# GuyTevet/motion-diffusion-model

Measured on AMD Instinct MI355X. Metric: motions/sec (B=128, T=196, 50-step DDPM), higher is better.
Workload: dtype f16x3 (fp32 operands split into fp16 hi+lo, 3 fp16 MFMA products, fp32 accumulate; everything else fp32); 1 GPU; HumanML3D text2motion, 50-step p_sample_loop with CFG 2.5 (2 denoiser forwards per step), batch=128 per GPU, T=196, 8-layer d=512 trans_enc MDM, random-init weights, cached text embedding; global_batch=128, diffusion_steps=50, parallelism=dp1: batch shards, no data-path collective, all_gather of final samples

## Files before the change

include/mdm_hip.h:

```cpp
#ifndef MDM_HIP_H
#define MDM_HIP_H

#include <stddef.h>
#include <stdint.h>

#ifdef __cplusplus
extern "C" {
#endif

#define MDM_OK 0
#define MDM_EINVAL (-1)
#define MDM_ESTATE (-2)
#define MDM_ENOSPC (-3)
#define MDM_EHIP (-4)
#define MDM_EUNSUPPORTED (-5)

#define MDM_ABI_VERSION 10

typedef struct mdm_model mdm_model_t;

#define MDM_ARCH_TRANS_ENC 0
#define MDM_ARCH_TRANS_DEC 1

typedef struct mdm_config {
// ... 3 lines not shown
  int32_t ff_size;
  int32_t num_layers;
  int32_t num_heads;
  int32_t clip_dim;
  int32_t max_len;
  int32_t mask_frames;
  int32_t arch;
  int32_t context_len;
} mdm_config_t;

int mdm_abi_version(void);
const char* mdm_build_info(void);
const char* mdm_last_error(void);

int mdm_create(const mdm_config_t* cfg, mdm_model_t** out);
void mdm_destroy(mdm_model_t* m);

#define MDM_OPT_SMALL_GEMM_MAX_SEQS 1
#define MDM_OPT_SMALL_GEMM_ROW_TILES 2
#define MDM_OPT_DEC_FUSED_XATTN 3
#define MDM_OPT_DEC_FUSED_SELFATTN 4
#define MDM_OPT_ATTN_DIRECT_OUT 5
#define MDM_OPT_DEC_TIME_TOKEN 6
int mdm_set_option(mdm_model_t* m, int32_t key, int32_t value);
int mdm_get_option(const mdm_model_t* m, int32_t key, int32_t* value);

int mdm_set_time_add(mdm_model_t* m, const float* add_dev, int32_t B);

int mdm_set_weight(mdm_model_t* m, const char* name, const float* dev_ptr, int64_t numel);

size_t mdm_const_bytes(const mdm_model_t* m);
int mdm_prepare(mdm_model_t* m, void* const_ws_dev, size_t const_ws_bytes, void* stream);

int mdm_weights_in_range(mdm_model_t* m, int32_t* in_range, void* stream);

#define MDM_PREC_F32 0
#define MDM_PREC_F16X3 1
int mdm_set_precision(mdm_model_t* m, int32_t mode);

size_t mdm_workspace_bytes(const mdm_model_t* m, int32_t nseq, int32_t nframes);

#define MDM_BRANCH_COND 0
#define MDM_BRANCH_UNCOND 1
#define MDM_BRANCH_BOTH 2

int mdm_forward(mdm_model_t* m, const float* x_dev, const int64_t* timesteps_dev, const float* text_embed_dev,
// ... 133 lines not shown
```

motion-diffusion-model_amd/_native.py:

```python
import ctypes as C
import os

_HERE = os.path.dirname(os.path.abspath(__file__))
LIB_NAME = "libmdm_hip.so"
LIB_PATH = os.path.join(_HERE, "csrc", LIB_NAME)
PROBE_LIB_PATH = os.path.join(_HERE, "csrc", "libmdm_hip_probe.so")

MDM_OK = 0
BRANCH_COND, BRANCH_UNCOND, BRANCH_BOTH = 0, 1, 2
ACT_NONE, ACT_GELU, ACT_SILU = 0, 1, 2
PRECISIONS = {"f32": 0, "f16x3": 1}
PROF_CLASSES = ("linear", "attention", "layernorm", "embed", "outproj", "elementwise")

EXPORTED_SYMBOLS = [
    "mdm_abi_version", "mdm_build_info", "mdm_last_error", "mdm_create", "mdm_destroy", "mdm_set_weight", "mdm_const_bytes",
    "mdm_prepare", "mdm_workspace_bytes", "mdm_forward", "mdm_sampler_step", "mdm_randn", "mdm_sample_loop",
    "mdm_linear", "mdm_layernorm", "mdm_attention", "mdm_profile_enable", "mdm_profile_read", "mdm_profile_reset",
    "mdm_set_precision", "mdm_linear_x3", "mdm_linear_x3_scratch_bytes", "mdm_attention_x3", "mdm_attention_x3_scratch_bytes",
    "mdm_recover_from_ric", "mdm_workspace_bytes_dec", "mdm_forward_dec", "mdm_workspace_bytes_dec_loop",
    "mdm_sample_loop_dec", "mdm_weights_in_range", "mdm_set_option", "mdm_get_option", "mdm_set_time_add",
    "mdm_rot6d_to_smpl_joints", "mdm_smpl_workspace_bytes", "mdm_smpl_forward",
]
PROBE_SYMBOLS = ["mdm_debug_set", "mdm_debug_get", "mdm_linear_f16f6", "mdm_linear_f16f6_scratch_bytes", "mdm_probe_in_proj"]
ABI_VERSION = 10
OPTIONS = {"small_gemm_max_seqs": 1, "small_gemm_row_tiles": 2, "dec_fused_xattn": 3, "dec_fused_selfattn": 4, "attn_direct_out": 5,
           "dec_time_token": 6}
ARCH = {"trans_enc": 0, "trans_dec": 1}


class MdmConfig(C.Structure):
    _fields_ = [(n, C.c_int32) for n in ("njoints", "nfeats", "latent_dim", "ff_size", "num_layers", "num_heads",
                                         "clip_dim", "max_len", "mask_frames", "arch", "context_len")]


class MdmSmplModel(C.Structure):
    _fields_ = [(n, C.c_void_p) for n in ("j0", "jdirs", "blend", "weights_t", "sel_blend", "sel_weights_t", "extra_t")] + \
               [("parents", C.POINTER(C.c_int32))] + [(n, C.c_int32) for n in ("J", "V", "n_sel", "n_extra")]


class MdmSmplCall(C.Structure):
    _fields_ = [(n, C.c_int32) for n in ("pose_rep", "glob", "translation", "vertstrans", "n_points", "root_point")] + \
               [("point_map", C.POINTER(C.c_int32)), ("glob_rot_mat", C.POINTER(C.c_float)), ("beta1", C.c_float)]


SMPL_POSE_REPS = {"rot6d": 0, "rotvec": 1, "rotmat": 2, "rotquat": 3}
SMPL_REP_FEATS = {"rot6d": 6, "rotvec": 3, "rotmat": 9, "rotquat": 4}


class MdmStep(C.Structure):
# ... 127 lines not shown
```

motion-diffusion-model_amd/csrc/api_launch.h:

```cpp
#pragma once

namespace {

struct Workspace {
  float *tok, *qkv, *att, *ffn, *cond;
  QkvPlanes qp;
  p16_t *xah, *xal;
  float *stat1, *stat2;
  p16_t *tokh, *tokl;
  p16_t *atth, *attl;
  p16_t *ffnh, *ffnl;
  size_t bytes;
};

Workspace carve(const mdm_model* m, int nseq, int T, void* base) {
  const size_t D = m->cfg.latent_dim, FF = m->cfg.ff_size, S = (size_t)T + 1, M = (size_t)nseq * S;
  size_t off = 0;
  auto take = [&](size_t floats) {
    size_t o = off;
    off += align_up(floats * sizeof(float), 256);
    return base ? reinterpret_cast<float*>(static_cast<char*>(base) + o) : nullptr;
  };
  Workspace w;
  w.tok = take(M * D);
// ... 217 lines not shown
    RowMajorLoader bl{w, K, N, K};
    launch_gemm_f32(al, bl, ep, M, N, K, s, x3);
  }
  return rt_launch_status();
}

int launch_linear_x3(Profiler* pf, X3Operand a, X3Weights w, const float* bias, const float* res, float* out,
                     p16_t* oh, p16_t* ol, int M, int N, int K, int act, int scale_cols, float col_scale, int seq_len,
                     hipStream_t s, X3Operand res_planes = X3Operand{nullptr, nullptr}) {
  if (K % X3_BK != 0) return fail(MDM_EINVAL, "f16x3 linear: K must be a multiple of 32");
  if (N % 4 != 0) return fail(MDM_EINVAL, "f16x3 linear: N must be a multiple of 4");
  ProfScope ps(pf, MDM_PROF_LINEAR, 2.0 * M * (double)N * K, s);
  X3Epilogue ep{out, bias, res, res_planes.hi, res_planes.lo, oh, ol, N, scale_cols, col_scale, QkvPlanes{}, 0, 0,
                nullptr, nullptr, nullptr, nullptr, nullptr, nullptr, 1, 1.f, 1, 1, 1};
#ifdef MDM_PROBES
  if (g_x3_delay > 1) ep.emb_B = g_x3_delay;
#endif
  const int rc = launch_gemm_x3(a, w, ep, M, N, K, act, seq_len, s, g_x3_ablate);
  if (rc == -2) return fail(MDM_EUNSUPPORTED, "f16x3 linear: unsupported (activation, residual, output) combination");
  return rt_launch_status();
}

int launch_in_proj_x3(Profiler* pf, X3Operand a, X3Weights w, const float* bias, const QkvPlanes& qp, int nseq, int S,
                      int D, float qscale, hipStream_t s) {
  if (D % X3_BK != 0) return fail(MDM_EINVAL, "f16x3 in_proj: latent_dim must be a multiple of 32");
  ProfScope ps(pf, MDM_PROF_LINEAR, 2.0 * nseq * S * 3.0 * D * (double)D, s);
  X3Epilogue ep{nullptr, bias, nullptr, nullptr, nullptr, nullptr, nullptr, 3 * D, D, qscale, qp, S, D,
                nullptr, nullptr, nullptr, nullptr, nullptr, nullptr, 1, 1.f, 1, 1, 1};
  const int rc = launch_gemm_x3_qkv(a, w, ep, nseq, S, D, s);
  if (rc == -2) return fail(MDM_EUNSUPPORTED, "f16x3 in_proj: sequences longer than 224 tokens");
  return rt_launch_status();
}

struct LnArgs {
  const float* astat = nullptr; const float* colsum = nullptr;
  X3Operand res{nullptr, nullptr}; const float* rstat = nullptr; const float* rgamma = nullptr; const float* rbeta = nullptr;
  float* ostat = nullptr;
  int parts = 1; float inv_dim = 1.f;
  const float* res_f32 = nullptr; int emb_T = 1, emb_B = 1, emb_nbranch = 1;
  bool small = false;
  X3sShape shape{1, 1};
  int stat_cols = 256;
};
inline bool use_small_gemm(const mdm_model* m, int nseq, int S) {
  return m->precision == MDM_PREC_F16X3 && m->lnfold && (nseq <= m->x3s.max_seqs || S > X3_TM) &&
         m->cfg.latent_dim % 128 == 0 && m->cfg.latent_dim % 256 == 0 && m->cfg.ff_size % 256 == 0;
}
int launch_x3_ln(Profiler* pf, int prof_cat, int kind, X3Operand a, X3Weights w, const float* bias, const LnArgs& ln,
                 float* out, p16_t* oh, p16_t* ol, const QkvPlanes* qp, int M, int N, int K, int S, int D,
                 int scale_cols, float col_scale, hipStream_t s) {
  if (K % X3_BK != 0 || N % 4 != 0) return fail(MDM_EINVAL, "f16x3 linear: K % 32 and N % 4 must be 0");
  if (ln.parts < 1 || ln.parts > (ln.small ? 8 : 4)) return fail(MDM_EUNSUPPORTED, "folded LayerNorm: too many partial sums per row (D <= 1024)");
  ProfScope ps(pf, prof_cat, 2.0 * M * (double)N * K, s);
// ... 52 lines not shown
```

motion-diffusion-model_amd/csrc/api_runtime.h:

```cpp
#pragma once

namespace {

thread_local std::string g_err;
#ifdef MDM_PROBES
int g_x3_ablate = 0;
int g_x3_reuse_planes = 0;
int g_f6_reference = 0;
int g_x3_delay = 0;
#else
constexpr int g_x3_ablate = 0, g_x3_reuse_planes = 0;
#endif

int fail(int code, const std::string& msg) {
  g_err = msg;
  return code;
}

#ifdef MDM_EMU
inline int rt_launch_status() { return 0; }
inline int rt_copy(void* dst, const void* src, size_t bytes, hipStream_t) { memcpy(dst, src, bytes); return 0; }
template <class K> inline int rt_allow_lds(K, size_t) { return 0; }
#else
inline int rt_launch_status() {
// ... 96 lines not shown
  const float* time_add_next = nullptr;
  int time_add_B = 0;
  const float* time_add = nullptr;
  bool dec_time_token = false;
  int jf = 0, jf_pad = 0;
  int precision = MDM_PREC_F16X3;
  struct LayerPlanes { X3Weights in_proj, out_proj, linear1, linear2; };
  std::vector<LayerPlanes> planes;
  struct LayerFold { X3Weights in_proj, linear1; float *c_qkv, *b_qkv, *c_1, *b_1; };
  std::vector<LayerFold> fold;
  struct DecFold { float *w_in, *c_in, *b_in, *w_q, *c_q, *b_q, *w_1, *c_1, *b_1; };
  std::vector<DecFold> dec_fold;
  struct DecPlanes { X3Weights in_proj, out_proj, q, out_proj2, linear1, linear2; };
  std::vector<DecPlanes> dec_planes;
  X3Weights in_planes{nullptr, nullptr};
  int jf_k = 0;
  X3Weights out_planes_f{nullptr, nullptr};
  float *c_out = nullptr, *b_out = nullptr;
  float *wkv_all = nullptr, *bkv_all = nullptr;
  bool lnfold = false;
  X3sOptions x3s;
  int fused_xattn = 3;
  bool fused_selfattn = true;
  bool attn_direct = false;
  X3Weights out_planes{nullptr, nullptr};
  float* out_bias_pad = nullptr;
  int jf_out = 0;

  const float* W(const std::string& k) const { return w.at(k); }
  const float* L(int layer, const char* suffix) const {
    return w.at((cfg.arch == MDM_ARCH_TRANS_DEC ? "seqTransDecoder.layers." : "seqTransEncoder.layers.") +
                std::to_string(layer) + "." + suffix);
  }
};

namespace {

#ifdef MDM_EMU
struct ChainGuard { explicit ChainGuard(void*) {} };
#else
struct DeviceChain {
  std::mutex mu;
  hipEvent_t ev = nullptr;
  hipStream_t last = nullptr;
  bool has = false;
};
// ... 57 lines not shown
```

motion-diffusion-model_amd/csrc/encoder.h:

```cpp
#pragma once

namespace {

int embed_frames_x3(mdm_model* m, const Workspace& ws, const float* x, int B, int T, int nbranch, hipStream_t s, const CondTokArgs& ct) {
  const int D = m->cfg.latent_dim, KP = m->jf_k;
  ProfScope ps(&m->prof, MDM_PROF_EMBED, 2.0 * B * T * (double)D * m->jf, s);
  p16_t* ph = reinterpret_cast<p16_t*>(ws.ffn);
  p16_t* pl = ph + (size_t)B * T * KP;
  MDM_LAUNCH(pose_planes_cond_kernel, dim3(((T + 31) / 32) * (KP / 32) * B + nbranch * B), dim3(256), 0, s, x, ph, pl, T, m->jf, KP, B, ct);
  if (int rc = rt_launch_status()) return rc;
  LnArgs a;
  a.res_f32 = m->W("sequence_pos_encoder.pe");
  a.emb_T = T; a.emb_B = B; a.emb_nbranch = nbranch;
  a.small = use_small_gemm(m, nbranch * B, T + 1) && KP == 288;
  a.shape = x3s_shape(m->x3s, nbranch * B);
  return launch_x3_ln(nullptr, MDM_PROF_EMBED, 5, X3Operand{ph, pl}, m->in_planes, m->W("input_process.poseEmbedding.bias"), a,
                      nullptr, ws.tokh, ws.tokl, nullptr, B * T, D, KP, T + 1, D, 0, 1.f, s);
}
inline bool use_embed_x3(const mdm_model* m, int T) {
  return m->precision == MDM_PREC_F16X3 && x3_waves_setting() == 8 &&
         (T + 1 <= X3_TM || (use_small_gemm(m, 1, T + 1) && m->jf_k == 288));
}

int embed_tokens(mdm_model* m, const Workspace& ws, const float* x, const long long* timesteps,
// ... 22 lines not shown
  return rt_launch_status();
}

int encoder(mdm_model* m, const Workspace& ws, int nseq, int B, int S, const int* lengths, hipStream_t s) {
  Profiler* pf = &m->prof;
  const int D = m->cfg.latent_dim, FF = m->cfg.ff_size, H = m->cfg.num_heads, M = nseq * S;
  const float qscale = 1.0f / sqrtf((float)(D / H));
  if (m->precision == MDM_PREC_F16X3 && m->lnfold && x3_waves_setting() == 8 && (S <= X3_TM || use_small_gemm(m, nseq, S))) {
    const X3Operand xb{ws.tokh, ws.tokl}, xa{ws.xah, ws.xal}, attp{ws.atth, ws.attl}, ffnp{ws.ffnh, ws.ffnl};
    const bool small = use_small_gemm(m, nseq, S);
    const X3sShape shape = x3s_shape(m->x3s, nseq);
    const int scols = small ? x3s_tn(shape.ncb) : 256;
    const int parts = (D + scols - 1) / scols;
    const float inv_dim = 1.0f / (float)D;
    auto LN = [&]() { LnArgs a; a.small = small; a.shape = shape; a.stat_cols = scols; a.parts = parts; a.inv_dim = inv_dim; return a; };
    for (int l = 0; l < m->cfg.num_layers; ++l) {
      const mdm_model::LayerPlanes& P = m->planes[l];
      const mdm_model::LayerFold& F = m->fold[l];
      if (l == 0 && small) {
        LnArgs a = LN();
        if (int rc = launch_x3_ln(pf, MDM_PROF_LINEAR, 6, xb, P.in_proj, m->L(l, "self_attn.in_proj_bias"), a, nullptr, nullptr,
                                  nullptr, &ws.qp, M, 3 * D, D, S, D, D, qscale, s)) return rc;
      } else if (l == 0) {
        if (int rc = launch_in_proj_x3(pf, xb, P.in_proj, m->L(l, "self_attn.in_proj_bias"), ws.qp, nseq, S, D, qscale, s)) return rc;
      } else {
        LnArgs a = LN(); a.astat = ws.stat2; a.colsum = F.c_qkv;
        if (int rc = launch_x3_ln(pf, MDM_PROF_LINEAR, 0, xb, F.in_proj, F.b_qkv, a, nullptr, nullptr, nullptr, &ws.qp, M,
                                  3 * D, D, S, D, D, qscale, s)) return rc;
      }
      if (int rc = launch_attention_x3(pf, ws.qp, lengths, nseq, B, S, D, nullptr, ws.atth, ws.attl, s, 1, m->attn_direct)) return rc;
      {
        LnArgs a = LN(); a.res = xb; a.ostat = ws.stat1;
        if (l >= 1) { a.rstat = ws.stat2; a.rgamma = m->L(l - 1, "norm2.weight"); a.rbeta = m->L(l - 1, "norm2.bias"); }
        if (int rc = launch_x3_ln(pf, MDM_PROF_LINEAR, l == 0 ? 1 : 2, attp, P.out_proj, m->L(l, "self_attn.out_proj.bias"),
                                  a, nullptr, ws.xah, ws.xal, nullptr, M, D, D, S, D, 0, 1.f, s)) return rc;
      }
      {
        LnArgs a = LN(); a.astat = ws.stat1; a.colsum = F.c_1;
        if (int rc = launch_x3_ln(pf, MDM_PROF_LINEAR, 3, xa, F.linear1, F.b_1, a, nullptr, ws.ffnh, ws.ffnl, nullptr, M, FF,
                                  D, S, D, 0, 1.f, s)) return rc;
      }
      {
        LnArgs a = LN(); a.res = xa; a.rstat = ws.stat1; a.rgamma = m->L(l, "norm1.weight"); a.rbeta = m->L(l, "norm1.bias");
        a.ostat = ws.stat2;
        if (int rc = launch_x3_ln(pf, MDM_PROF_LINEAR, 2, ffnp, P.linear2, m->L(l, "linear2.bias"), a, nullptr, ws.tokh,
                                  ws.tokl, nullptr, M, D, FF, S, D, 0, 1.f, s)) return rc;
      }
// ... 60 lines not shown
```

motion-diffusion-model_amd/csrc/gemm_x3.h:

```cpp
#pragma once
#include "attention_x3.h"
#include "common.h"
#include "gemm_f32.h"
#include <cstdlib>

namespace mdm {

constexpr int X3_TM = 224, X3_BK = 32;
constexpr int x3_tn(int waves) { return 32 * waves; }
constexpr int X3_MSUB = X3_TM / 32;
constexpr int X3_A_BYTES = X3_TM * X3_BK * 2;
constexpr int X3_A_STAGE = 2 * X3_A_BYTES;
constexpr int X3_A_RING = 2;
constexpr int X3_PIPE_RING = 4;
#ifndef MDM_X3_EPI_AHEAD
#define MDM_X3_EPI_AHEAD 0
#endif
constexpr bool X3_EPI_AHEAD = MDM_X3_EPI_AHEAD != 0;
#ifdef MDM_X3_PIPE_BADWAIT
constexpr int X3P_MID_SLACK = 8;
#else
constexpr int X3P_MID_SLACK = 0;
#endif
#if defined(MDM_X3_PIPE_WDRAIN)
constexpr int X3P_WAIT_WS = 0, X3P_WAIT_MID = 0;
#elif defined(MDM_X3_PIPE_STRICT)
constexpr int X3P_WAIT_WS = 6, X3P_WAIT_MID = 3;
#else
constexpr int X3P_WAIT_WS = 12, X3P_WAIT_MID = 7;
#endif
#if defined(MDM_X3_PIPE_WDRAIN)
// ... 34 lines not shown
  float* out;
  const float* bias;
  const float* res;
  const p16_t* resh;
  const p16_t* resl;
  p16_t* oh;
  p16_t* ol;
  int ld;
  int scale_cols;
  float col_scale;
  QkvPlanes qkv;
  int S, D;
  const float* astat;
  const float* colsum;
  const float* rstat;
  const float* rgamma;
  const float* rbeta;
  float* ostat;
  int stat_parts;
  float inv_dim;
  int emb_T, emb_B, emb_nbranch;
  float acc_scale = kX3AccScale;
  int stat_cols = 256;
};

constexpr bool x3_has_col_scale(int act, int res) { return act == 0 && (res == 0 || res == 1); }

__device__ __forceinline__ float gelu_erf_fast(float x) {
  const float z = fabsf(x) * 0.70710678118654752440f;
#ifdef MDM_EMU
  const float t = 1.0f / (1.0f + 0.3275911f * z);
#else
  const float t = __builtin_amdgcn_rcpf(1.0f + 0.3275911f * z);
#endif
  float p = 1.061405429f;
  p = p * t - 1.453152027f;
  p = p * t + 1.421413741f;
  p = p * t - 0.284496736f;
  p = p * t + 0.254829592f;
#ifdef MDM_EMU
  const float erfc_z = p * t * expf(-z * z);
#else
  const float erfc_z = p * t * __expf(-z * z);
#endif
  const float erf_abs = 1.0f - erfc_z;
  return 0.5f * x * (1.0f + copysignf(erf_abs, x));
// ... 28 lines not shown

constexpr int x3_res_rounds(int t, bool t16) { return (t16 && t == X3_MSUB - 1) ? 2 : 4; }
constexpr int x3_res_younger_rounds(int t, int rr, bool t16) {
  int n = 0;
  for (int q = t + 1; q <= t + rr - 1 && q < X3_MSUB; ++q) n += x3_res_rounds(q, t16);
  return n;
}

#if !defined(MDM_EMU) && defined(MDM_PROBES)
#define MDM_X3_DBG 1
__device__ unsigned long long g_x3_dbg[8];
__device__ __forceinline__ unsigned long long x3_now() { return __builtin_readcyclecounter(); }
#endif

template <int PIECES>
struct X3Cursor {
  int v;
  int k;
  uint32_t off[PIECES];
};

template <int WAVES, int ACT, int RES, bool OUT_F32, bool OUT_PLANES, bool OUT_QKV, int ABL, bool FOLD = false,
          bool OSTAT = false, bool EMBED = false, bool T16 = false, bool F6 = false, bool PIPE = false, int NCB = 1,
          bool M16 = false>
__global__ __launch_bounds__(64 * WAVES, NCB == 2 ? 1 : 2) void gemm_x3_kernel(X3Operand A, X3Weights W, X3Epilogue ep, int M, int N,
                                                                     int K, int rows_per_tile, int tiles_n, int total) {
  MDM_DYN_SMEM(unsigned char, lds);
  static_assert(!PIPE || (T16 && (WAVES == 8 || (WAVES == 4 && NCB == 2)) && !F6), "the pipelined k-loop exists for 208-row (T16), 256-column tiles");
  static_assert(NCB == 1 || (NCB == 2 && PIPE && WAVES == 4), "two column blocks per wave: the pipelined 4-wave form only");
  static_assert(!M16 || (PIPE && WAVES == 8 && NCB == 1 && ABL == 0), "the 16x16x32 form: pipelined, 8 waves, no ablations");
  constexpr int RINGN = PIPE ? X3_PIPE_RING : X3_A_RING;
  constexpr int NBLK = WAVES * NCB;
  constexpr int X3_WAVES = WAVES, X3_TN = 32 * NBLK, X3_A_PIECES = x3_a_pieces(WAVES);
  constexpr int NT32 = T16 ? X3_MSUB - 1 : X3_MSUB;
  constexpr int NROUNDS = 4 * NT32 + (T16 ? 2 : 0);
  using Cursor = X3Cursor<X3_A_PIECES>;

  const int tid = threadIdx.x;
  const int lane = tid & 63;
#ifdef MDM_EMU
  const int wid = tid >> 6;
#else
  const int wid = __builtin_amdgcn_readfirstlane(tid >> 6);
#endif
  const int r = lane & 31, h = lane >> 5;
  const int nk = K / X3_BK;
  const int gstride = (int)gridDim.x;

  auto tile_origin = [&](int v, int& m0, int& n0) {
    const int lid = xcd_remap(v, total);
    const int tile_m = lid / tiles_n, tile_n = lid - tile_m * tiles_n;
    m0 = tile_m * rows_per_tile;
    n0 = tile_n * X3_TN;
  };

  const int schunk = (lane & 3) ^ ((lane >> 4) & 3);
  auto aim_a = [&](Cursor& c) {
    int m0, n0;
    tile_origin(c.v, m0, n0);
#pragma unroll
    for (int i = 0; i < X3_A_PIECES; ++i) {
      const int jj = min(wid + X3_WAVES * i, 25);
      const int q = PIPE ? (jj < 13 ? jj : jj + 1) : min(wid + X3_WAVES * i, X3_A_GROUPS - 1);
      const int ga = (q < 14) ? q : q - 14;
      const int arow = min(m0 + ga * 16 + (lane >> 2), M - 1);
      if constexpr ((ABL & 16) != 0) {
        c.off[i] = (uint32_t)(arow >> 4) * (uint32_t)(K / 32) * 512u + (uint32_t)(arow & 15) * 32u + schunk * 8;
      } else {
        c.off[i] = (uint32_t)arow * (uint32_t)K + schunk * 8;
      }
    }
  };
  auto piece_a = [&](const Cursor& c, int i, int buf) {
    if constexpr (PIPE) {
      const int j = wid + X3_WAVES * i;
      const int q = j < 13 ? j : j + 1;
      if (j < 26) glds16(((q < 14) ? A.hi : A.lo) + c.off[i] + c.k * X3_BK, lds + buf * X3_A_STAGE + q * 1024);
    } else {
      const int q = wid + X3_WAVES * i;
      if (q < X3_A_GROUPS && !(T16 && (q == 13 || q == 27)))
        glds16(((q < 14) ? A.hi : A.lo) + c.off[i] + c.k * ((ABL & 16) ? 512 : X3_BK), lds + buf * X3_A_STAGE + q * 1024);
    }
  };
  auto advance_a = [&](Cursor& c) {
    if (++c.k == nk) {
      c.k = 0;
      if (c.v + gstride < total) { c.v += gstride; aim_a(c); }
    }
  };

  const size_t wk16 = (size_t)(K / 16);
  auto load_w = [&](int v, int k, p16x8 (&fh)[2], p16x8 (&fl)[2]) {
    int m0, n0;
    tile_origin(v, m0, n0);
    const size_t nb = (size_t)((n0 >> 5) + wid);
    const size_t o = ((nb * wk16 + 2 * (size_t)k) * 64 + lane) * 8;
    fh[0] = *reinterpret_cast<const p16x8*>(W.hi + o);
    fl[0] = *reinterpret_cast<const p16x8*>(W.lo + o);
    fh[1] = *reinterpret_cast<const p16x8*>(W.hi + o + 512);
    fl[1] = *reinterpret_cast<const p16x8*>(W.lo + o + 512);
  };

  const int sw = (r >> 2) & 3;
  const int fa = r * 64;
  const int r16 = lane & 15, g16 = lane >> 4;
  const int fa16 = (192 + r16) * 64 + ((g16 ^ ((r16 >> 2) & 3)) * 16);
#ifndef MDM_EMU
  const uint32_t lds_base = lds_addr_of(lds);
#endif

  int v = (int)blockIdx.x;
  if (v >= total) return;
#if defined(MDM_PROBES) && !defined(MDM_EMU)
  if constexpr (WAVES == 4 && !EMBED) {
    if (ep.emb_B > 1 && (int)blockIdx.x >= gstride / 2) {
      const unsigned long long t0 = __builtin_readcyclecounter();
      while (__builtin_readcyclecounter() - t0 < (unsigned long long)ep.emb_B * 64ULL) __builtin_amdgcn_s_sleep(8);
    }
  }
#endif
  Cursor ca{v, 0, {}};
  aim_a(ca);
  int wv = v, wkk = 0;

  auto stats_dma = [&](int m0s, int par) {
    const float* st = FOLD ? ep.astat : ep.rstat;
    const int npieces = (X3_TM * ep.stat_parts * 8 + 1023) / 1024;
    for (int pc = wid; pc < npieces; pc += X3_WAVES) {
      const long long total_f = (long long)M * ep.stat_parts * 2;
// ... 590 lines not shown
      }
    };

    if (OUT_QKV) {
      const int Dm = ep.D, SPq = ep.qkv.SP, Hq = ep.qkv.H;
      int ncol_e = ncol0, m0_e = m0;
#ifndef MDM_EMU
      asm volatile("" : "+s"(ncol_e), "+s"(m0_e));
#endif
      const int which = ncol_e / Dm, hcol = ncol_e - which * Dm, head = hcol >> 7, d0 = hcol & 127;
      const size_t shq = (size_t)(m0_e / rows_per_tile) * Hq + head;
      if (ncol0 < N && !(ABL & 1)) {
        if (which == 2) {
          p16_t* vhp = ep.qkv.vh + ((shq * ep.qkv.NKT) * AX_HD + d0 + r) * 32 + 8 * h;
          p16_t* vlp = ep.qkv.vl + ((shq * ep.qkv.NKT) * AX_HD + d0 + r) * 32 + 8 * h;
          const int nkt = ep.qkv.NKT;
          if constexpr (M16) {
#pragma unroll
            for (int cb = 0; cb < 2; ++cb) {
              const int cl = 16 * cb + r16;
              const float b16 = cvec[wblk * 32 + cl];
              const float c16 = FOLD ? cvec[256 + wblk * 32 + cl] : 0.f;
              const size_t o0 = (shq * ep.qkv.NKT * AX_HD + d0 + cl) * 32 + 4 * ((g16 >> 1) + 2 * (g16 & 1));
#pragma unroll
              for (int s = 0; s < NS16; ++s) {
                if ((s >> 1) < nkt) {
                  float vv[4];
#pragma unroll
                  for (int e = 0; e < 4; ++e) {
                    if constexpr (FOLD) {
                      const float2 st = atab[16 * s + 4 * g16 + e];
                      vv[e] = st.y * (accm_[s][cb][e] * accs - st.x * c16) + b16;
                    } else {
                      vv[e] = accm_[s][cb][e] * accs + b16;
                    }
                  }
                  const size_t o = o0 + (size_t)(s >> 1) * (AX_HD * 32) + 16 * (s & 1);
                  split4_store(ep.qkv.vh + o, ep.qkv.vl + o, make_float4(vv[0], vv[1], vv[2], vv[3]));
                }
              }
            }
          } else {
#pragma unroll
          for (int t = 0; t < NT32; ++t) {
            if (t < nkt) {
#pragma unroll
              for (int s2 = 0; s2 < 2; ++s2) {
                float vv[8];
#pragma unroll
                for (int j = 0; j < 8; ++j) {
                  if constexpr (FOLD) {
                    const float2 st = atab[32 * t + mfma_row(8 * s2 + j, h)];
                    vv[j] = st.y * (acc[t][8 * s2 + j] * accs - st.x * csum) + bias;
                  } else {
                    vv[j] = acc[t][8 * s2 + j] * accs + bias;
                  }
                }
                p16x8 vh8, vl8;
                split8(vv, vh8, vl8);
                *reinterpret_cast<p16x8*>(vhp + t * (AX_HD * 32) + 16 * s2) = vh8;
                *reinterpret_cast<p16x8*>(vlp + t * (AX_HD * 32) + 16 * s2) = vl8;
// ... 6 lines not shown
              for (int cb = 0; cb < 2; ++cb) {
                const int cl = 16 * cb + r16;
                const float b16 = lane_bcast(bias, cl);
                const float c16 = FOLD ? lane_bcast(csum, cl) : 0.f;
                float vv[4];
#pragma unroll
                for (int e = 0; e < 4; ++e) {
                  if constexpr (FOLD) {
                    const float2 st = atab[192 + 4 * g16 + e];
                    vv[e] = st.y * (acc16[cb][e] * accs - st.x * c16) + b16;
                  } else {
                    vv[e] = acc16[cb][e] * accs + b16;
                  }
                }
                const size_t o = ((shq * ep.qkv.NKT + NT32) * AX_HD + d0 + cl) * 32 + 4 * ((g16 >> 1) + 2 * (g16 & 1));
                split4_store(ep.qkv.vh + o, ep.qkv.vl + o, make_float4(vv[0], vv[1], vv[2], vv[3]));
              }
            }
          }
          }
        } else {
          p16_t* dh = (which == 0 ? ep.qkv.qh : ep.qkv.kh) + shq * SPq * AX_HD + d0 + pc4;
          p16_t* dl = (which == 0 ? ep.qkv.ql : ep.qkv.kl) + shq * SPq * AX_HD + d0 + pc4;
          const int nkt = ep.qkv.NKT;
          patch_write(std::integral_constant<int, 0>{});
          float2 st_cur = row_stats(std::integral_constant<int, 0>{});
          float4 v_cur = zero4();
          if constexpr (X3_EPI_AHEAD) {
            wave_lds_fence();
            v_cur = ld4(&patch[prow * 32 + pc4]);
            wave_lds_fence();
            patch_write(std::integral_constant<int, 1>{});
          }
          static_for<NROUNDS>([&](auto j_tag) __attribute__((always_inline)) {
            constexpr int j = decltype(j_tag)::value, t = j / 4, g = j % 4;
            float4 v4;
            float2 st_next;
            if constexpr (X3_EPI_AHEAD) {
              wave_lds_fence();
              float4 v_next = zero4();
              if constexpr (j + 1 < NROUNDS) v_next = ld4(&patch[prow * 32 + pc4]);
              st_next = row_stats(std::integral_constant<int, j + 1>{});
              wave_lds_fence();
              patch_write(std::integral_constant<int, j + 2>{});
              v4 = v_cur;
              v_cur = v_next;
            } else {
              wave_lds_fence();
              v4 = ld4(&patch[prow * 32 + pc4]);
              st_next = row_stats(std::integral_constant<int, j + 1>{});
              wave_lds_fence();
              patch_write(std::integral_constant<int, j + 1>{});
            }
            const float2 st = st_cur;
            st_cur = st_next;
            if (t < nkt) {
              const int tok = 32 * t + 8 * g + prow;
              v4 = finish4(v4, st);
              if (t < X3_MSUB - 1 || tok < ep.S) split4_store(dh + tok * AX_HD, dl + tok * AX_HD, v4);
            }
          });
        }
      }
    } else {
      constexpr bool HAS_RES = RES != 0;
      constexpr bool RES_PLANES = RES == 2 || RES == 3;
      static_assert(!(EMBED && RES_PLANES), "the EMBED epilogue takes an fp32 residual");
      constexpr bool CLIP_OUT = OUT_PLANES && !EMBED;
      const uint32_t pitch2 = (uint32_t)ep.ld * 2u;
      const uint32_t voff0 = n4 < N ? ((uint32_t)prow * (uint32_t)ep.ld + (uint32_t)n4) * 2u : CLIP_OFF;
      ClipWin w_oh = {}, w_ol = {}, w_rh = {}, w_rl = {};
      {
        int m0_e = m0;
#ifndef MDM_EMU
        asm volatile("" : "+s"(m0_e));
#endif
        const size_t row0 = (size_t)m0_e * ep.ld;
        if constexpr (CLIP_OUT) {
          const uint32_t bytes = (uint32_t)(m_end - m0_e) * pitch2;
          w_oh = clip_win(ep.oh + row0, bytes);
          w_ol = clip_win(ep.ol + row0, bytes);
        }
// ... 190 lines not shown
  int wgs = per_cu * cus / 8 * 8;
#ifdef MDM_PROBES
  static const int div = [] { const char* e = getenv("MDM_X3_GRID_DIV"); return e != nullptr && atoi(e) > 1 ? atoi(e) : 1; }();
  wgs = wgs / div / 8 * 8;
#endif
  return wgs > 0 ? wgs : 8;
#endif
}

#ifdef MDM_PROBES
inline int& x3_waves_setting() {
  static int waves = [] {
    const char* e = getenv("MDM_X3_WAVES");
    return (e != nullptr && e[0] == '4') ? 4 : 8;
  }();
  return waves;
}
#else
inline int x3_waves_setting() { return 8; }
#endif

template <int WAVES, int ACT, int RES, bool OUT_F32, bool OUT_PLANES, bool OUT_QKV, int ABL, bool FOLD = false,
          bool OSTAT = false, bool EMBED = false, bool T16 = false, bool F6 = false, bool PIPE = false, int NCB = 1,
          bool M16 = false>
inline int launch_gemm_x3_w(const X3Operand& A, const X3Weights& W, const X3Epilogue& ep, int M, int N, int K,
                                int rpt, hipStream_t stream) {
  constexpr int NBLK = WAVES * NCB;
  constexpr int TN = 32 * NBLK;
  constexpr bool LN = FOLD || OSTAT || RES == 3;
  constexpr int RINGN = PIPE ? X3_PIPE_RING : X3_A_RING;
  const int tiles_m = (M + rpt - 1) / rpt, tiles_n = (N + TN - 1) / TN;
  const int total = tiles_m * tiles_n;
  static_assert(!(F6 && T16), "the f16f6 k-loop has no 16-row sub-tile yet");
  auto kfn = &gemm_x3_kernel<WAVES, ACT, RES, OUT_F32, OUT_PLANES, OUT_QKV, ABL, FOLD, OSTAT, EMBED, T16, F6, PIPE, NCB, M16>;
  if (T16 && rpt > X3_TM - 16) return -2;
  if (PIPE && (K / X3_BK) % 2 != 0) return -2;
  if (!x3_has_col_scale(ACT, RES) && ep.scale_cols > 0) return -2;
#ifndef MDM_EMU
  if (x3_lds_bytes(NBLK, LN, RINGN) > 65536) {
    static bool configured[kMaxDevices] = {};
    if (const int rc = rt_dyn_lds_once(kfn, x3_lds_bytes(NBLK, LN, RINGN), configured, stream)) return rc;
  }
#endif
  const int grid = std::min(total, x3_grid_limit((WAVES == 4 && NCB == 1) ? 2 : 1));
  MDM_LAUNCH(kfn, dim3(grid), dim3(64 * WAVES), x3_lds_bytes(NBLK, LN, RINGN), stream, A, W, ep, M, N, K, rpt, tiles_n, total);
  return 0;
}

inline bool x3_wide_setting() {
#ifdef MDM_PROBES
  const char* e = getenv("MDM_X3_WIDE");
  return e != nullptr && e[0] == '1';
#else
  return false;
#endif
}

inline bool x3_pipe_setting(int kind = 0) {
// ... 141 lines not shown
  if (act == ACT_GELU && !res && !f32 && pl) return launch_gemm_x3_t<ACT_GELU, 0, false, true, false>(A, W, ep, M, N, K, rpt, s);
  if (act == ACT_GELU && !res && f32 && !pl) return launch_gemm_x3_t<ACT_GELU, 0, true, false, false>(A, W, ep, M, N, K, rpt, s);
  if (act == ACT_GELU && res && f32 && !pl) return launch_gemm_x3_t<ACT_GELU, 1, true, false, false>(A, W, ep, M, N, K, rpt, s);
  if (act == ACT_SILU && !res && f32 && !pl) return launch_gemm_x3_t<ACT_SILU, 0, true, false, false>(A, W, ep, M, N, K, rpt, s);
  return -2;
}

#ifdef MDM_PROBES
inline int launch_gemm_f16f6(const X3Operand& A, const X3Weights& W, const X3Epilogue& ep, int M, int N, int K, int act,
                             hipStream_t s) {
  const bool res = ep.res != nullptr;
  if (act == ACT_NONE && !res && x3_waves_setting() == 4)
    return launch_gemm_x3_w<4, ACT_NONE, 0, true, false, false, 0, false, false, false, false, true>(A, W, ep, M, N, K, X3_TM, s);
  if (act == ACT_NONE && !res)
    return launch_gemm_x3_w<8, ACT_NONE, 0, true, false, false, 0, false, false, false, false, true>(A, W, ep, M, N, K, X3_TM, s);
  if (act == ACT_NONE && res)
    return launch_gemm_x3_w<8, ACT_NONE, 1, true, false, false, 0, false, false, false, false, true>(A, W, ep, M, N, K, X3_TM, s);
  if (act == ACT_GELU && !res)
    return launch_gemm_x3_w<8, ACT_GELU, 0, true, false, false, 0, false, false, false, false, true>(A, W, ep, M, N, K, X3_TM, s);
  return -2;
}
#endif

inline int launch_gemm_x3_qkv(const X3Operand& A, const X3Weights& W, const X3Epilogue& ep, int nseq, int S, int D,
                                  hipStream_t s) {
  if (S > X3_TM) return -2;
  if (x3_waves_setting() == 8 && S <= X3_TM - 16 && x3_t16_setting()) {
    if ((D / X3_BK) % 2 == 0 && x3_pipe_setting(5)) {
#ifdef MDM_PROBES
      if (x3_wide_setting())
        return launch_gemm_x3_w<4, ACT_NONE, 0, false, false, true, 0, false, false, false, true, false, true, 2>(A, W, ep, nseq * S,
                                                                                                                   3 * D, D, S, s);
      if (!x3_m16_setting())
        return launch_gemm_x3_w<8, ACT_NONE, 0, false, false, true, 0, false, false, false, true, false, true>(A, W, ep, nseq * S,
                                                                                                                3 * D, D, S, s);
#endif
      return launch_gemm_x3_w<8, ACT_NONE, 0, false, false, true, 0, false, false, false, true, false, true, 1, true>(
          A, W, ep, nseq * S, 3 * D, D, S, s);
    }
    return launch_gemm_x3_w<8, ACT_NONE, 0, false, false, true, 0, false, false, false, true>(A, W, ep, nseq * S, 3 * D, D,
                                                                                                 S, s);
  }
  return launch_gemm_x3_t<ACT_NONE, 0, false, false, true>(A, W, ep, nseq * S, 3 * D, D, S, s);
}

#endif

}
```

motion-diffusion-model_amd/csrc/mdm_api.hip:

```cpp
#include "../../include/mdm_hip.h"
#ifdef MDM_PROBES
#include "../../include/mdm_hip_probe.h"
#endif

#include <algorithm>
#include <cmath>
#include <cstdio>
#include <cstring>
#include <map>
#include <mutex>
#include <new>
#include <string>
#include <vector>

#include "attention_x3.h"
#include "attention_long.h"
#include "attention_f32.h"
#include "common.h"
#include "elementwise.h"
#include "gemm_f32.h"
#include "gemm_x3.h"
#include "gemm_x3s.h"
#include "xattn_block.h"
#include "selfattn_block.h"
// ... 119 lines not shown
      return MDM_OK;
    case MDM_OPT_SMALL_GEMM_ROW_TILES:
      if (value < 0 || value > 2) return fail(MDM_EINVAL, "mdm_set_option: MDM_OPT_SMALL_GEMM_ROW_TILES must be 0 (by size), 1 or 2");
      m->x3s.row_tiles = value;
      return MDM_OK;
    case MDM_OPT_DEC_FUSED_XATTN:
      if (value < 0 || value > 3) return fail(MDM_EINVAL, "mdm_set_option: MDM_OPT_DEC_FUSED_XATTN must be 0, 1, 2 or 3");
      m->fused_xattn = value;
      return MDM_OK;
    case MDM_OPT_DEC_FUSED_SELFATTN:
      if (value != 0 && value != 1) return fail(MDM_EINVAL, "mdm_set_option: MDM_OPT_DEC_FUSED_SELFATTN must be 0 or 1");
      m->fused_selfattn = value != 0;
      return MDM_OK;
    case MDM_OPT_ATTN_DIRECT_OUT:
      if (value != 0 && value != 1) return fail(MDM_EINVAL, "mdm_set_option: MDM_OPT_ATTN_DIRECT_OUT must be 0 or 1");
      m->attn_direct = value != 0;
      return MDM_OK;
    case MDM_OPT_DEC_TIME_TOKEN:
      if (value != 0 && value != 1) return fail(MDM_EINVAL, "mdm_set_option: MDM_OPT_DEC_TIME_TOKEN must be 0 or 1");
      if (value == 1 && (m->cfg.arch != MDM_ARCH_TRANS_DEC || m->cfg.context_len != 1))
        return fail(MDM_EINVAL, "mdm_set_option: MDM_OPT_DEC_TIME_TOKEN needs a trans_dec model created with context_len = 1 (the class-token row)");
      m->dec_time_token = value != 0;
      return MDM_OK;
    default:
      return fail(MDM_EINVAL, "mdm_set_option: unknown key " + std::to_string(key));
  }
}

int mdm_set_time_add(mdm_model_t* m, const float* add_dev, int32_t B) {
  if (m == nullptr) return fail(MDM_EINVAL, "mdm_set_time_add: null model");
  if (add_dev != nullptr && B <= 0) return fail(MDM_EINVAL, "mdm_set_time_add: B must be >= 1");
  m->time_add_next = add_dev;
  m->time_add_B = add_dev != nullptr ? B : 0;
  return MDM_OK;
}

int mdm_get_option(const mdm_model_t* m, int32_t key, int32_t* value) {
  if (m == nullptr || value == nullptr) return fail(MDM_EINVAL, "mdm_get_option: null argument");
  switch (key) {
    case MDM_OPT_SMALL_GEMM_MAX_SEQS: *value = m->x3s.max_seqs; return MDM_OK;
    case MDM_OPT_SMALL_GEMM_ROW_TILES: *value = m->x3s.row_tiles; return MDM_OK;
    case MDM_OPT_DEC_FUSED_XATTN: *value = m->fused_xattn; return MDM_OK;
    case MDM_OPT_DEC_FUSED_SELFATTN: *value = m->fused_selfattn ? 1 : 0; return MDM_OK;
    case MDM_OPT_ATTN_DIRECT_OUT: *value = m->attn_direct ? 1 : 0; return MDM_OK;
    case MDM_OPT_DEC_TIME_TOKEN: *value = m->dec_time_token ? 1 : 0; return MDM_OK;
    default: return fail(MDM_EINVAL, "mdm_get_option: unknown key " + std::to_string(key));
  }
}

int mdm_set_weight(mdm_model_t* m, const char* name, const float* dev_ptr, int64_t numel) {
  if (m == nullptr || name == nullptr || dev_ptr == nullptr) return fail(MDM_EINVAL, "mdm_set_weight: null argument");
  auto it = m->expect.find(name);
  if (it == m->expect.end()) return fail(MDM_EINVAL, std::string("unexpected state-dict key: ") + name);
  if (it->second != numel)
    return fail(MDM_EINVAL, std::string("size mismatch for ") + name + ": expected " + std::to_string(it->second) +
                                " elements, got " + std::to_string(numel));
  if ((reinterpret_cast<uintptr_t>(dev_ptr) & 15) != 0) return fail(MDM_EINVAL, std::string(name) + ": pointer must be 16-byte aligned");
  m->w[name] = dev_ptr;
  m->prepared = false;
  return MDM_OK;
}

size_t mdm_const_bytes(const mdm_model_t* m) {
  if (m == nullptr) return 0;
  const size_t D = m->cfg.latent_dim;
  const size_t FF = m->cfg.ff_size;
  if (m->cfg.arch == MDM_ARCH_TRANS_DEC) {
    const size_t fold = align_up(3 * D * D * 4, 256) + align_up(D * D * 4, 256) + align_up(FF * D * 4, 256) +
// ... 751 lines not shown
```

Measured before the change: 396.5 motions/s.

## Share layer-0 QKV projection between CFG cond and uncond branches

In the encoder's first layer the cond and uncond sequences differ only in the first (condition) token, so the QKV in_proj runs once over B sequences with one extra row that holds the uncond token. It then writes both branches' Q/K/V planes, shifting and replacing token 0 for the paired copy. This roughly halves the layer-0 in_proj GEMM work, at the cost of a more complex epilogue with duplicated stores and a lane broadcast. The LDS A-stage swizzle is also changed to a new permutation.

```diff
diff --git a/include/mdm_hip.h b/include/mdm_hip.h
--- a/include/mdm_hip.h
+++ b/include/mdm_hip.h
@@ -49,6 +49,7 @@
 #define MDM_OPT_DEC_FUSED_SELFATTN 4
 #define MDM_OPT_ATTN_DIRECT_OUT 5
 #define MDM_OPT_DEC_TIME_TOKEN 6
+#define MDM_OPT_ENC_SHARED_LAYER0 7
 int mdm_set_option(mdm_model_t* m, int32_t key, int32_t value);
 int mdm_get_option(const mdm_model_t* m, int32_t key, int32_t* value);
 
diff --git a/motion-diffusion-model_amd/_native.py b/motion-diffusion-model_amd/_native.py
--- a/motion-diffusion-model_amd/_native.py
+++ b/motion-diffusion-model_amd/_native.py
@@ -24,7 +24,7 @@
 PROBE_SYMBOLS = ["mdm_debug_set", "mdm_debug_get", "mdm_linear_f16f6", "mdm_linear_f16f6_scratch_bytes", "mdm_probe_in_proj"]
 ABI_VERSION = 10
 OPTIONS = {"small_gemm_max_seqs": 1, "small_gemm_row_tiles": 2, "dec_fused_xattn": 3, "dec_fused_selfattn": 4, "attn_direct_out": 5,
-           "dec_time_token": 6}
+           "dec_time_token": 6, "enc_shared_layer0": 7}
 ARCH = {"trans_enc": 0, "trans_dec": 1}
 
 
diff --git a/motion-diffusion-model_amd/csrc/api_launch.h b/motion-diffusion-model_amd/csrc/api_launch.h
--- a/motion-diffusion-model_amd/csrc/api_launch.h
+++ b/motion-diffusion-model_amd/csrc/api_launch.h
@@ -263,13 +263,15 @@
 }
 
 int launch_in_proj_x3(Profiler* pf, X3Operand a, X3Weights w, const float* bias, const QkvPlanes& qp, int nseq, int S,
-                      int D, float qscale, hipStream_t s) {
+                      int D, float qscale, hipStream_t s, int pair_B = 0) {
   if (D % X3_BK != 0) return fail(MDM_EINVAL, "f16x3 in_proj: latent_dim must be a multiple of 32");
-  ProfScope ps(pf, MDM_PROF_LINEAR, 2.0 * nseq * S * 3.0 * D * (double)D, s);
+  const double rows = pair_B > 0 ? (double)pair_B * (S + 1) : (double)nseq * S;
+  ProfScope ps(pf, MDM_PROF_LINEAR, 2.0 * rows * 3.0 * D * (double)D, s);
   X3Epilogue ep{nullptr, bias, nullptr, nullptr, nullptr, nullptr, nullptr, 3 * D, D, qscale, qp, S, D,
                 nullptr, nullptr, nullptr, nullptr, nullptr, nullptr, 1, 1.f, 1, 1, 1};
-  const int rc = launch_gemm_x3_qkv(a, w, ep, nseq, S, D, s);
-  if (rc == -2) return fail(MDM_EUNSUPPORTED, "f16x3 in_proj: sequences longer than 224 tokens");
+  const int rc = launch_gemm_x3_qkv(a, w, ep, nseq, S, D, s, pair_B);
+  if (rc == -2) return fail(MDM_EUNSUPPORTED, pair_B > 0 ? "f16x3 in_proj: the paired layer-0 launch does not cover this shape"
+                                                         : "f16x3 in_proj: sequences longer than 224 tokens");
   return rt_launch_status();
 }
 
diff --git a/motion-diffusion-model_amd/csrc/api_runtime.h b/motion-diffusion-model_amd/csrc/api_runtime.h
--- a/motion-diffusion-model_amd/csrc/api_runtime.h
+++ b/motion-diffusion-model_amd/csrc/api_runtime.h
@@ -142,6 +142,7 @@
   X3sOptions x3s;
   int fused_xattn = 3;
   bool fused_selfattn = true;
+  bool enc_shared_l0 = true;
   bool attn_direct = false;
   X3Weights out_planes{nullptr, nullptr};
   float* out_bias_pad = nullptr;
diff --git a/motion-diffusion-model_amd/csrc/encoder.h b/motion-diffusion-model_amd/csrc/encoder.h
--- a/motion-diffusion-model_amd/csrc/encoder.h
+++ b/motion-diffusion-model_amd/csrc/encoder.h
@@ -68,7 +68,8 @@
         if (int rc = launch_x3_ln(pf, MDM_PROF_LINEAR, 6, xb, P.in_proj, m->L(l, "self_attn.in_proj_bias"), a, nullptr, nullptr,
                                   nullptr, &ws.qp, M, 3 * D, D, S, D, D, qscale, s)) return rc;
       } else if (l == 0) {
-        if (int rc = launch_in_proj_x3(pf, xb, P.in_proj, m->L(l, "self_attn.in_proj_bias"), ws.qp, nseq, S, D, qscale, s)) return rc;
+        const int pair_B = (m->enc_shared_l0 && nseq == 2 * B && x3_qkv_pairs(S, D)) ? B : 0;
+        if (int rc = launch_in_proj_x3(pf, xb, P.in_proj, m->L(l, "self_attn.in_proj_bias"), ws.qp, nseq, S, D, qscale, s, pair_B)) return rc;
       } else {
         LnArgs a = LN(); a.astat = ws.stat2; a.colsum = F.c_qkv;
         if (int rc = launch_x3_ln(pf, MDM_PROF_LINEAR, 0, xb, F.in_proj, F.b_qkv, a, nullptr, nullptr, nullptr, &ws.qp, M,
diff --git a/motion-diffusion-model_amd/csrc/gemm_x3.h b/motion-diffusion-model_amd/csrc/gemm_x3.h
--- a/motion-diffusion-model_amd/csrc/gemm_x3.h
+++ b/motion-diffusion-model_amd/csrc/gemm_x3.h
@@ -7,6 +7,8 @@
 namespace mdm {
 
 constexpr int X3_TM = 224, X3_BK = 32;
+__host__ __device__ constexpr int x3_swz(int q) { return (((q ^ (q >> 1)) & 1) << 1) | (q >> 1); }
+static_assert(x3_swz(0) == 0 && x3_swz(1) == 2 && x3_swz(2) == 3 && x3_swz(3) == 1, "A-stage swizzle permutation");
 constexpr int x3_tn(int waves) { return 32 * waves; }
 constexpr int X3_MSUB = X3_TM / 32;
 constexpr int X3_A_BYTES = X3_TM * X3_BK * 2;
@@ -87,6 +89,7 @@
   int emb_T, emb_B, emb_nbranch;
   float acc_scale = kX3AccScale;
   int stat_cols = 256;
+  int pair_B = 0;
 };
 
 constexpr bool x3_has_col_scale(int act, int res) { return act == 0 && (res == 0 || res == 1); }
@@ -161,13 +164,14 @@
 
 template <int WAVES, int ACT, int RES, bool OUT_F32, bool OUT_PLANES, bool OUT_QKV, int ABL, bool FOLD = false,
           bool OSTAT = false, bool EMBED = false, bool T16 = false, bool F6 = false, bool PIPE = false, int NCB = 1,
-          bool M16 = false>
+          bool M16 = false, bool PAIR = false>
 __global__ __launch_bounds__(64 * WAVES, NCB == 2 ? 1 : 2) void gemm_x3_kernel(X3Operand A, X3Weights W, X3Epilogue ep, int M, int N,
                                                                      int K, int rows_per_tile, int tiles_n, int total) {
   MDM_DYN_SMEM(unsigned char, lds);
   static_assert(!PIPE || (T16 && (WAVES == 8 || (WAVES == 4 && NCB == 2)) && !F6), "the pipelined k-loop exists for 208-row (T16), 256-column tiles");
   static_assert(NCB == 1 || (NCB == 2 && PIPE && WAVES == 4), "two column blocks per wave: the pipelined 4-wave form only");
   static_assert(!M16 || (PIPE && WAVES == 8 && NCB == 1 && ABL == 0), "the 16x16x32 form: pipelined, 8 waves, no ablations");
+  static_assert(!PAIR || (M16 && OUT_QKV && !FOLD), "the paired tile: layer 0's in_proj (no folded LayerNorm) on the 16x16x32 form");
   constexpr int RINGN = PIPE ? X3_PIPE_RING : X3_A_RING;
   constexpr int NBLK = WAVES * NCB;
   constexpr int X3_WAVES = WAVES, X3_TN = 32 * NBLK, X3_A_PIECES = x3_a_pieces(WAVES);
@@ -193,7 +197,7 @@
     n0 = tile_n * X3_TN;
   };
 
-  const int schunk = (lane & 3) ^ ((lane >> 4) & 3);
+  const int schunk = (lane & 3) ^ x3_swz((lane >> 4) & 3);
   auto aim_a = [&](Cursor& c) {
     int m0, n0;
     tile_origin(c.v, m0, n0);
@@ -202,7 +206,10 @@
       const int jj = min(wid + X3_WAVES * i, 25);
       const int q = PIPE ? (jj < 13 ? jj : jj + 1) : min(wid + X3_WAVES * i, X3_A_GROUPS - 1);
       const int ga = (q < 14) ? q : q - 14;
-      const int arow = min(m0 + ga * 16 + (lane >> 2), M - 1);
+      int arow = min(m0 + ga * 16 + (lane >> 2), M - 1);
+      if constexpr (PAIR) {
+        if (ga * 16 + (lane >> 2) == rows_per_tile) arow = m0 + M;
+      }
       if constexpr ((ABL & 16) != 0) {
         c.off[i] = (uint32_t)(arow >> 4) * (uint32_t)(K / 32) * 512u + (uint32_t)(arow & 15) * 32u + schunk * 8;
       } else {
@@ -240,10 +247,10 @@
     fl[1] = *reinterpret_cast<const p16x8*>(W.lo + o + 512);
   };
 
-  const int sw = (r >> 2) & 3;
+  const int sw = x3_swz((r >> 2) & 3);
   const int fa = r * 64;
   const int r16 = lane & 15, g16 = lane >> 4;
-  const int fa16 = (192 + r16) * 64 + ((g16 ^ ((r16 >> 2) & 3)) * 16);
+  const int fa16 = (192 + r16) * 64 + ((g16 ^ x3_swz((r16 >> 2) & 3)) * 16);
 #ifndef MDM_EMU
   const uint32_t lds_base = lds_addr_of(lds);
 #endif
@@ -880,6 +887,21 @@
               const float b16 = cvec[wblk * 32 + cl];
               const float c16 = FOLD ? cvec[256 + wblk * 32 + cl] : 0.f;
               const size_t o0 = (shq * ep.qkv.NKT * AX_HD + d0 + cl) * 32 + 4 * ((g16 >> 1) + 2 * (g16 & 1));
+              auto vfin = [&](float a) __attribute__((always_inline)) { return a * accs + b16; };
+              float u0 = 0.f;
+              size_t po = 0;
+              if constexpr (PAIR) {
+                const int sS = ep.S >> 4, eS = ep.S & 3;
+#pragma unroll
+                for (int s = 0; s < NS16; ++s) {
+                  if (s == sS) {
+                    const f32x4 a = accm_[s][cb];
+                    u0 = vfin(eS == 0 ? a[0] : eS == 1 ? a[1] : eS == 2 ? a[2] : a[3]);
+                  }
+                }
+                u0 = lane_bcast(u0, r16 + 16 * ((ep.S >> 2) & 3));
+                po = (size_t)ep.pair_B * Hq * ep.qkv.NKT * (AX_HD * 32);
+              }
 #pragma unroll
               for (int s = 0; s < NS16; ++s) {
                 if ((s >> 1) < nkt) {
@@ -890,11 +912,15 @@
                       const float2 st = atab[16 * s + 4 * g16 + e];
                       vv[e] = st.y * (accm_[s][cb][e] * accs - st.x * c16) + b16;
                     } else {
-                      vv[e] = accm_[s][cb][e] * accs + b16;
+                      vv[e] = vfin(accm_[s][cb][e]);
                     }
                   }
                   const size_t o = o0 + (size_t)(s >> 1) * (AX_HD * 32) + 16 * (s & 1);
                   split4_store(ep.qkv.vh + o, ep.qkv.vl + o, make_float4(vv[0], vv[1], vv[2], vv[3]));
+                  if constexpr (PAIR) {
+                    const float k0 = (s == 0 && g16 == 0) ? u0 : vv[0];
+                    split4_store(ep.qkv.vh + po + o, ep.qkv.vl + po + o, make_float4(k0, vv[1], vv[2], vv[3]));
+                  }
                 }
               }
             }
@@ -947,7 +973,8 @@
         } else {
           p16_t* dh = (which == 0 ? ep.qkv.qh : ep.qkv.kh) + shq * SPq * AX_HD + d0 + pc4;
           p16_t* dl = (which == 0 ? ep.qkv.ql : ep.qkv.kl) + shq * SPq * AX_HD + d0 + pc4;
-          const int nkt = ep.qkv.NKT;
+          const int nkt = PAIR ? (ep.S + 32) / 32 : ep.qkv.NKT;
+          const size_t pq = PAIR ? (size_t)ep.pair_B * Hq * SPq * AX_HD : 0;
           patch_write(std::integral_constant<int, 0>{});
           float2 st_cur = row_stats(std::integral_constant<int, 0>{});
           float4 v_cur = zero4();
@@ -982,7 +1009,15 @@
             if (t < nkt) {
               const int tok = 32 * t + 8 * g + prow;
               v4 = finish4(v4, st);
-              if (t < X3_MSUB - 1 || tok < ep.S) split4_store(dh + tok * AX_HD, dl + tok * AX_HD, v4);
+              if constexpr (PAIR) {
+                if (tok < ep.S) split4_store(dh + tok * AX_HD, dl + tok * AX_HD, v4);
+                if ((unsigned)(tok - 1) < (unsigned)ep.S) {
+                  const int tok2 = tok == ep.S ? 0 : tok;
+                  split4_store(dh + pq + tok2 * AX_HD, dl + pq + tok2 * AX_HD, v4);
+                }
+              } else {
+                if (t < X3_MSUB - 1 || tok < ep.S) split4_store(dh + tok * AX_HD, dl + tok * AX_HD, v4);
+              }
             }
           });
         }
@@ -1219,7 +1254,7 @@
 
 template <int WAVES, int ACT, int RES, bool OUT_F32, bool OUT_PLANES, bool OUT_QKV, int ABL, bool FOLD = false,
           bool OSTAT = false, bool EMBED = false, bool T16 = false, bool F6 = false, bool PIPE = false, int NCB = 1,
-          bool M16 = false>
+          bool M16 = false, bool PAIR = false>
 inline int launch_gemm_x3_w(const X3Operand& A, const X3Weights& W, const X3Epilogue& ep, int M, int N, int K,
                                 int rpt, hipStream_t stream) {
   constexpr int NBLK = WAVES * NCB;
@@ -1229,8 +1264,9 @@
   const int tiles_m = (M + rpt - 1) / rpt, tiles_n = (N + TN - 1) / TN;
   const int total = tiles_m * tiles_n;
   static_assert(!(F6 && T16), "the f16f6 k-loop has no 16-row sub-tile yet");
-  auto kfn = &gemm_x3_kernel<WAVES, ACT, RES, OUT_F32, OUT_PLANES, OUT_QKV, ABL, FOLD, OSTAT, EMBED, T16, F6, PIPE, NCB, M16>;
+  auto kfn = &gemm_x3_kernel<WAVES, ACT, RES, OUT_F32, OUT_PLANES, OUT_QKV, ABL, FOLD, OSTAT, EMBED, T16, F6, PIPE, NCB, M16, PAIR>;
   if (T16 && rpt > X3_TM - 16) return -2;
+  if (PAIR && (rpt + 1 > X3_TM - 16 || ep.pair_B < 1 || M != ep.pair_B * rpt)) return -2;
   if (PIPE && (K / X3_BK) % 2 != 0) return -2;
   if (!x3_has_col_scale(ACT, RES) && ep.scale_cols > 0) return -2;
 #ifndef MDM_EMU
@@ -1418,9 +1454,21 @@
 }
 #endif
 
+inline bool x3_qkv_pairs(int S, int D) {
+  return x3_waves_setting() == 8 && S + 1 <= X3_TM - 16 && x3_t16_setting() && (D / X3_BK) % 2 == 0 && x3_pipe_setting(5) &&
+         !x3_wide_setting() && x3_m16_setting();
+}
+
 inline int launch_gemm_x3_qkv(const X3Operand& A, const X3Weights& W, const X3Epilogue& ep, int nseq, int S, int D,
-                                  hipStream_t s) {
+                                  hipStream_t s, int pair_B = 0) {
   if (S > X3_TM) return -2;
+  if (pair_B > 0) {
+    if (nseq != 2 * pair_B || !x3_qkv_pairs(S, D)) return -2;
+    X3Epilogue ep2 = ep;
+    ep2.pair_B = pair_B;
+    return launch_gemm_x3_w<8, ACT_NONE, 0, false, false, true, 0, false, false, false, true, false, true, 1, true, true>(
+        A, W, ep2, pair_B * S, 3 * D, D, S, s);
+  }
   if (x3_waves_setting() == 8 && S <= X3_TM - 16 && x3_t16_setting()) {
     if ((D / X3_BK) % 2 == 0 && x3_pipe_setting(5)) {
 #ifdef MDM_PROBES
diff --git a/motion-diffusion-model_amd/csrc/mdm_api.hip b/motion-diffusion-model_amd/csrc/mdm_api.hip
--- a/motion-diffusion-model_amd/csrc/mdm_api.hip
+++ b/motion-diffusion-model_amd/csrc/mdm_api.hip
@@ -165,6 +165,10 @@
         return fail(MDM_EINVAL, "mdm_set_option: MDM_OPT_DEC_TIME_TOKEN needs a trans_dec model created with context_len = 1 (the class-token row)");
       m->dec_time_token = value != 0;
       return MDM_OK;
+    case MDM_OPT_ENC_SHARED_LAYER0:
+      if (value != 0 && value != 1) return fail(MDM_EINVAL, "mdm_set_option: MDM_OPT_ENC_SHARED_LAYER0 must be 0 or 1");
+      m->enc_shared_l0 = value != 0;
+      return MDM_OK;
     default:
       return fail(MDM_EINVAL, "mdm_set_option: unknown key " + std::to_string(key));
   }
@@ -187,6 +191,7 @@
     case MDM_OPT_DEC_FUSED_SELFATTN: *value = m->fused_selfattn ? 1 : 0; return MDM_OK;
     case MDM_OPT_ATTN_DIRECT_OUT: *value = m->attn_direct ? 1 : 0; return MDM_OK;
     case MDM_OPT_DEC_TIME_TOKEN: *value = m->dec_time_token ? 1 : 0; return MDM_OK;
+    case MDM_OPT_ENC_SHARED_LAYER0: *value = m->enc_shared_l0 ? 1 : 0; return MDM_OK;
     default: return fail(MDM_EINVAL, "mdm_get_option: unknown key " + std::to_string(key));
   }
 }
```

Measured after the change: 401.4 motions/s, median of 6. 1.01x the previous value.
